# ViliamVadocz/takzero

Measured on NVIDIA B200. Metric: self-play MCTS simulations/sec, 6x6 Tak, higher is better.
Workload: dtype f16

## Files before the change

### takzero_b200/csrc/conv_tcgen05.cuh

```cuda
#pragma once
#include <cuda_bf16.h>
#include <cuda_fp16.h>
#include <stdint.h>
#include <stdio.h>

#include "encode.cuh"

namespace conv {

constexpr int TILE_M = 128;
constexpr int HALO = 8;
constexpr int A_ROWS = TILE_M + 2 * HALO;
constexpr int A_KC_BYTES = A_ROWS * 16;
constexpr int A_STAGE_BYTES = 8 * A_KC_BYTES;
#ifndef TZ_A_STAGES
#define TZ_A_STAGES 4
#endif
#ifndef TZ_B_STAGES
#define TZ_B_STAGES 8
#endif
constexpr int A_STAGES = TZ_A_STAGES;
constexpr int B_KC_BYTES = 128 * 16;
constexpr int B_STAGE_BYTES = 8 * B_KC_BYTES;
constexpr int B_STAGES = TZ_B_STAGES;
constexpr int N_OUT = 256;
constexpr int THREADS = 256;
constexpr int W_EPI0 = 0, W_APROD = 4, W_BPROD = 5, W_MMA = 6, W_ALLOC = 7;
constexpr int MASK_BYTES = 37 * 9 * 16;
constexpr int GATHER_BYTES = 4 * 32 * 32 * 4;
constexpr int SMEM_BYTES =
    A_STAGES * A_STAGE_BYTES + B_STAGES * B_STAGE_BYTES + 4096  + 512  +
    MASK_BYTES + GATHER_BYTES;
static_assert(SMEM_BYTES <= 227 * 1024, "shared memory budget of one CTA");
constexpr int MAX_LAYERS = 48;

struct Layer {
    const __nv_bfloat16* in;
    const TzState* enc_states;
    const __nv_bfloat16* w;
    const float* bias;
    const __nv_bfloat16* residual;
    __nv_bfloat16* out_act;
    const float* head_w;
    float* head_out;
    float* g_out;
    const uint16_t* g_actions;
    const uint32_t* g_ranges;
    const uint16_t* g_perm;
    int g_stride;
    int cin;
    int relu;
    int out_is_residual;
};

struct Params {
    Layer layers[MAX_LAYERS];
    const __nv_bfloat16* dead_after[MAX_LAYERS];
    int n_layers;
    long long rows_set;
    long long set_stride;
    int chunk_min_tiles;
    const int* count_ptr;
    int count_max;
    int n;
    int guard;
    const uint4* masks;
    int f16;
    unsigned* progress;
    unsigned* chunk_done;
    unsigned* status;
    int debug_drop_progress;
    int allow_local;
    int pack;
};

struct Item {
    int chunk, layer, pt;
    int tiles;
    int rows;
};
struct Schedule {
    int chunk_rows;
    int chunk_tiles;
    int rows_used;
    int n_layers;
    int items;
    __host__ __device__ __forceinline__ void init(int count, int nn, int chunk_min_tiles, int layers) {
        rows_used = count * nn;
        const int c1 = count > 0 ? count : 1;
        const int all_tiles = (rows_used + 2 * TILE_M - 1) / (2 * TILE_M);
        const int n_chunks = all_tiles >= 2 * chunk_min_tiles ? all_tiles / chunk_min_tiles : 1;
        const int cp = (c1 + n_chunks - 1) / n_chunks;
        chunk_rows = cp * nn;
        chunk_tiles = (chunk_rows + 2 * TILE_M - 1) / (2 * TILE_M);
        n_layers = layers;
        const int full = rows_used / chunk_rows, rest = rows_used - full * chunk_rows;
        items = (full * chunk_tiles + (rest + 2 * TILE_M - 1) / (2 * TILE_M)) * layers;
// ... 20 lines not shown
    return t;
}
#define CHAIN(cond, layer, kind, k)                                        \
    do {                                                                   \
        if (cond) g_chain[((layer) - 10) * 32 + (kind) * 4 + (k)] = gtime(); \
    } while (0)
#else
#define CHAIN(cond, layer, kind, k)
#endif

#ifdef TZ_DEBUG_TIMING
#define TWAIT(acc, stmt)                 \
    do {                                 \
        const long long t0_ = clock64(); \
        stmt;                            \
        acc += clock64() - t0_;          \
    } while (0)
#else
#define TWAIT(acc, stmt) stmt
#endif

__device__ __forceinline__ uint32_t smem_u32(const void* p) { return (uint32_t)__cvta_generic_to_shared(p); }

__device__ __forceinline__ bool row_position(int pack, int nn, int count, unsigned row, int* q, int* sq) {
    if (pack == 0) {
        *q = (int)(row / (unsigned)nn);
        *sq = (int)(row - (unsigned)*q * (unsigned)nn);
        return true;
    }
    const unsigned tile = row / (unsigned)TILE_M, w = row - tile * (unsigned)TILE_M, b = w / (unsigned)nn;
    *q = (int)(tile * (unsigned)pack + b);
    *sq = (int)(w - b * (unsigned)nn);
    return (int)b < pack && *q < count;
}

__device__ __forceinline__ void mbar_init(uint32_t bar, uint32_t count) {
    asm volatile("mbarrier.init.shared::cta.b64 [%0], %1;" ::"r"(bar), "r"(count));
}
__device__ __forceinline__ void mbar_wait(uint32_t bar, uint32_t parity) {
    asm volatile(
        "{\n\t"
        ".reg .pred p;\n\t"
        "WAIT_%=:\n\t"
        "mbarrier.try_wait.parity.shared::cta.b64 p, [%0], %1;\n\t"
        "@p bra DONE_%=;\n\t"
        "bra WAIT_%=;\n\t"
        "DONE_%=:\n\t"
        "}\n" ::"r"(bar),
        "r"(parity)
        : "memory");
}
__device__ __forceinline__ void mbar_arrive(uint32_t bar) {
    asm volatile("mbarrier.arrive.shared::cta.b64 _, [%0];" ::"r"(bar) : "memory");
}
__device__ __forceinline__ void mbar_arrive_n(uint32_t bar, uint32_t n) {
    asm volatile("mbarrier.arrive.shared::cta.b64 _, [%0], %1;" ::"r"(bar), "r"(n) : "memory");
// ... 106 lines not shown
    asm volatile(
        "tcgen05.commit.cta_group::2.mbarrier::arrive::one.shared::cluster.multicast::cluster.b64 [%0], %1;" ::"r"(bar),
        "h"((uint16_t)3)
        : "memory");
}
__device__ __forceinline__ void tc_mma_pair(uint32_t tmem_d, uint64_t adesc, uint64_t bdesc, uint32_t idesc, uint32_t acc,
                                            const uint4& m0, const uint4& m1) {
    asm volatile(
        "{\n\t"
        ".reg .pred p;\n\t"
        "setp.ne.b32 p, %4, 0;\n\t"
        "tcgen05.mma.cta_group::2.kind::f16 [%0], %1, %2, %3, {%5, %6, %7, %8, %9, %10, %11, %12}, p;\n\t"
        "}\n" ::"r"(tmem_d),
        "l"(adesc), "l"(bdesc), "r"(idesc), "r"(acc), "r"(m0.x), "r"(m0.y), "r"(m0.z), "r"(m0.w), "r"(m1.x), "r"(m1.y),
        "r"(m1.z), "r"(m1.w)
        : "memory");
}


__global__ void __cluster_dims__(2, 1, 1) __launch_bounds__(THREADS, 1) k_conv3x3_pair(const __grid_constant__ Params p) {
    extern __shared__ __align__(128) uint8_t smem[];
    const int warp = threadIdx.x >> 5, lane = threadIdx.x & 31;
    const uint32_t rank = cluster_rank();
    uint8_t* a_smem = smem;
    uint8_t* b_smem = smem + A_STAGES * A_STAGE_BYTES;
    float* s_bias = reinterpret_cast<float*>(b_smem + B_STAGES * B_STAGE_BYTES);
    uint64_t* bars = reinterpret_cast<uint64_t*>(reinterpret_cast<uint8_t*>(s_bias) + 4096);
    const uint32_t bar0 = smem_u32(bars);
    const uint32_t a_full = bar0, a_land = a_full + 8 * A_STAGES, a_empty = a_land + 8 * A_STAGES;
    const uint32_t b_full = a_empty + 8 * A_STAGES, b_land = b_full + 8 * B_STAGES;
    const uint32_t b_empty = b_land + 8 * B_STAGES;
    const uint32_t t_full = b_empty + 8 * B_STAGES, t_empty = t_full + 16;
    uint32_t* tmem_slot = reinterpret_cast<uint32_t*>(bars + 3 * A_STAGES + 3 * B_STAGES + 4);
    uint4* s_masks = reinterpret_cast<uint4*>(reinterpret_cast<uint8_t*>(bars) + 512);
    float* s_gather = reinterpret_cast<float*>(reinterpret_cast<uint8_t*>(s_masks) + MASK_BYTES);

    const int count = p.count_ptr ? *p.count_ptr : p.count_max;
    const int nn = p.n * p.n;
    const int period = p.pack ? TILE_M : nn;
    Schedule sched;
    sched.init(p.pack ? (count + p.pack - 1) / p.pack : count, period, p.chunk_min_tiles, p.n_layers);
    const int items = sched.items;
    const int pair = blockIdx.x >> 1, npairs = gridDim.x >> 1;
    const bool fine = sched.chunk_tiles < 2 * npairs;
    const bool local = p.allow_local && p.n_layers > 1 && (TILE_M % period) == 0 && sched.chunk_tiles <= npairs &&
                       items == sched.chunk_tiles * p.n_layers;
    const int item0 = local ? (pair < sched.chunk_tiles ? pair : items) : pair;
    const int istep = local ? sched.chunk_tiles : npairs;
    const uint32_t a_arrivals = local ? 4u : 1u;

    if (threadIdx.x == 0) {
        for (int i = 0; i < A_STAGES; i++) {
            mbar_init(a_full + 8 * i, 2 * a_arrivals);
            mbar_init(a_land + 8 * i, 1);
            mbar_init(a_empty + 8 * i, 1);
        }
        for (int i = 0; i < B_STAGES; i++) {
            mbar_init(b_full + 8 * i, 2);
            mbar_init(b_land + 8 * i, 1);
            mbar_init(b_empty + 8 * i, 1);
        }
        for (int i = 0; i < 2; i++) {
            mbar_init(t_full + 8 * i, 1);
            mbar_init(t_empty + 8 * i, 8);
        }
        asm volatile("fence.mbarrier_init.release.cluster;" ::: "memory");
    }
    if (warp == W_ALLOC) {
        asm volatile("tcgen05.alloc.cta_group::2.sync.aligned.shared::cta.b32 [%0], %1;" ::"r"(smem_u32(tmem_slot)),
                     "r"(512)
                     : "memory");
        asm volatile("tcgen05.relinquish_alloc_permit.cta_group::2.sync.aligned;" ::: "memory");
    }
    for (int i = threadIdx.x; i < (nn + 1) * 9; i += THREADS) s_masks[i] = p.masks[i];
    tc_fence_before();
    __syncthreads();
    cluster_sync_all();
    tc_fence_after();
    const uint32_t tmem_base = *tmem_slot;
    const uint32_t a_sig = rank == 0 ? a_full : a_land, b_sig = rank == 0 ? b_full : b_land;

    if (warp == W_APROD) {
        int stage = 0, phase = 0;
        for (int item = item0; item < items; item += istep) {
            const Item it = sched.at(item);
            const int layer = it.layer, pt = it.pt;
            const Layer& L = p.layers[layer];
            const int t = pt * 2 + (int)rank;
            if (L.enc_states != nullptr) {
                if (lane == 0) {
                    if (it.chunk >= 2 && p.n_layers > 1)
                        wait_counter(p.chunk_done + it.chunk - 2, 8u * (unsigned)sched.chunk_tiles, p.status);
                    mbar_wait(a_empty + 8 * stage, phase ^ 1);
                }
                __syncwarp();
#ifdef TZ_DEBUG_TIMING
                const long long enc_t0 = clock64();
#endif
                uint8_t* dst = a_smem + stage * A_STAGE_BYTES;
                const int first = t * TILE_M - HALO;
                constexpr int RPL = (A_ROWS + 31) / 32;
                uint64_t stack[RPL];
                uint4 tail[RPL];
                uint32_t hts[RPL];
#pragma unroll
                for (int k = 0; k < RPL; k++) {
                    const int r = lane + 32 * k;
                    const int rel = first + r;
                    hts[k] = 0xffffffffu;
                    stack[k] = 0;
                    tail[k] = make_uint4(0u, 0u, 0u, 0u);
                    if (r < A_ROWS && rel >= 0 && rel < it.rows) {
                        const unsigned grow = (unsigned)(it.chunk * sched.chunk_rows + rel);
                        int q, sq;
                        if (row_position(p.pack, nn, count, grow, &q, &sq)) {
                            const uint8_t* st = reinterpret_cast<const uint8_t*>(L.enc_states + q);
                            stack[k] = *reinterpret_cast<const uint64_t*>(st + 8 * sq);
                            hts[k] = (uint32_t)st[288 + sq] | ((uint32_t)st[324 + sq] << 8) | ((uint32_t)st[360] << 16);
                            tail[k] = *reinterpret_cast<const uint4*>(st + 368);
                        }
                    }
                }
#pragma unroll
                for (int k = 0; k < RPL; k++) {
                    const int r = lane + 32 * k;
                    if (r >= A_ROWS) continue;
                    uint8_t* row = dst + r * 16;
                    if (hts[k] != 0xffffffffu) {
                        const uint64_t ones = enc::square_indicator_bits(stack[k], (int)(hts[k] & 0xff), (int)((hts[k] >> 8) & 0xff),
                                                                         (int)((hts[k] >> 16) & 0xff), p.n);
                        enc::encode_square16_smem(row, A_KC_BYTES, ones, tail[k].y, tail[k].z, tail[k].w, p.n, p.f16);
                    } else {
#pragma unroll
                        for (int kc = 0; kc < 8; kc++) *reinterpret_cast<uint4*>(row + kc * A_KC_BYTES) = make_uint4(0u, 0u, 0u, 0u);
                    }
                }
                asm volatile("fence.proxy.async.shared::cta;" ::: "memory");
                __syncwarp();
                if (lane == 0) {
                    if (rank == 0) mbar_arrive_n(a_sig + 8 * stage, a_arrivals);
                    else mbar_arrive(a_sig + 8 * stage);
                }
#ifdef TZ_DEBUG_TIMING
                if (pair == 0 && rank == 0 && lane == 0 && item < 2 * npairs) printf("encode of one tile: %lld cycles\n", clock64() - enc_t0);
#endif
                if (++stage == A_STAGES) {
                    stage = 0;
                    phase ^= 1;
                }
                continue;
            }
            const int kblocks = L.cin >> 6;
            if (local) continue;
            if (lane == 0) {
                const unsigned need = 8u * (unsigned)layer;
                const unsigned* prog = p.progress + ((size_t)it.chunk * sched.chunk_tiles) * 4;
                const int lo = pt - 1 + (int)rank;
                const __nv_bfloat16* in_base = L.in + (size_t)(it.chunk & 1) * p.set_stride;
                const uint8_t* src_tile =
                    reinterpret_cast<const uint8_t*>(in_base) + (size_t)(p.guard + t * TILE_M - HALO) * 16;
                int st = stage, ph = phase;
                for (int kb = 0; kb < kblocks; kb++) {
                    if (layer > 0 && (fine || kb == 0)) {
                        const int blk = fine ? kb : 3;
                        for (int q = lo; q <= lo + 1; q++)
                            if (q >= 0 && q < it.tiles) wait_counter(prog + q * 4 + blk, need, p.status);
                        fence_proxy_async();
                        CHAIN(pair == 10 && rank == 0 && (layer == 10 || layer == 11), layer, 0, kb);
                    }
                    mbar_wait(a_empty + 8 * st, ph ^ 1);
                    mbar_arrive_expect_tx(a_sig + 8 * st, A_STAGE_BYTES);
                    const uint32_t dst = smem_u32(a_smem + st * A_STAGE_BYTES);
#pragma unroll
                    for (int kc = 0; kc < 8; kc++)
                        bulk_g2s(dst + kc * A_KC_BYTES, src_tile + (size_t)(kb * 8 + kc) * (size_t)p.rows_set * 16,
                                 A_KC_BYTES, a_sig + 8 * st);
                    if (++st == A_STAGES) {
                        st = 0;
                        ph ^= 1;
                    }
                }
            }
            for (int kb = 0; kb < kblocks; kb++)
                if (++stage == A_STAGES) {
                    stage = 0;
                    phase ^= 1;
                }
        }
    } else if (warp == W_BPROD) {
        if (lane == 0) {
            int stage = 0, phase = 0;
            for (int item = item0; item < items; item += istep) {
                const Layer& L = p.layers[sched.at(item).layer];
                const uint8_t* src = reinterpret_cast<const uint8_t*>(L.w) + (size_t)rank * B_STAGE_BYTES;
                const int blocks = (L.cin >> 6) * 9;
                for (int blk = 0; blk < blocks; blk++) {
                    mbar_wait(b_empty + 8 * stage, phase ^ 1);
                    mbar_arrive_expect_tx(b_sig + 8 * stage, B_STAGE_BYTES);
                    bulk_g2s(smem_u32(b_smem + stage * B_STAGE_BYTES), src + (size_t)blk * 2 * B_STAGE_BYTES,
                             B_STAGE_BYTES, b_sig + 8 * stage);
                    if (++stage == B_STAGES) {
                        stage = 0;
                        phase ^= 1;
                    }
                }
            }
        }
    } else if (warp == W_ALLOC) {
        if (rank != 0 && lane == 0) {
            int stage = 0, phase = 0;
            const uint32_t b_full_leader = map_to_rank(b_full, 0);
            for (int item = item0; item < items; item += istep) {
                const int blocks = (p.layers[sched.at(item).layer].cin >> 6) * 9;
                for (int blk = 0; blk < blocks; blk++) {
                    mbar_wait(b_land + 8 * stage, phase);
                    mbar_arrive_cluster(b_full_leader + 8 * stage);
                    if (++stage == B_STAGES) {
                        stage = 0;
                        phase ^= 1;
                    }
                }
            }
        }
    } else if (warp == W_MMA) {
        if (rank != 0) {
            if (lane == 0) {
                int stage = 0, phase = 0;
                const uint32_t a_full_leader = map_to_rank(a_full, 0);
                for (int item = item0; item < items; item += istep) {
                    const Layer& RL = p.layers[sched.at(item).layer];
                    if (local && RL.enc_states == nullptr) break;
                    const int kblocks = RL.cin >> 6;
                    for (int kb = 0; kb < kblocks; kb++) {
                        mbar_wait(a_land + 8 * stage, phase);
                        mbar_arrive_cluster_n(a_full_leader + 8 * stage, a_arrivals);
                        if (++stage == A_STAGES) {
                            stage = 0;
                            phase ^= 1;
                        }
                    }
                }
            }
        } else {
            const uint32_t fmt = p.f16 ? 0u : 1u;
            const uint32_t idesc = (1u << 4) | (fmt << 7) | (fmt << 10) | ((uint32_t)(N_OUT >> 3) << 17) |
                                   ((uint32_t)((2 * TILE_M) >> 4) << 24);
            int a_stage = 0, a_phase = 0, b_stage = 0, b_phase = 0, it = 0;
#ifdef TZ_DEBUG_TIMING
            long long w_t = 0, w_a = 0, w_b = 0, w_a0 = 0;
            const long long mma_start = clock64();
            long long gt_start;
            asm volatile("mov.u64 %0, %%globaltimer;" : "=l"(gt_start));
#endif
            for (int item = item0; item < items; item += istep, it++) {
                const Item wi = sched.at(item);
                const int pt = wi.pt;
                const int kblocks = p.layers[wi.layer].cin >> 6;
                const int acc = it & 1;
                TWAIT(w_t, mbar_wait(t_empty + 8 * acc, ((it >> 1) & 1) ^ 1));
                tc_fence_after();
                const uint32_t tmem_d = tmem_base + acc * N_OUT;
                const uint4* masks0 = s_masks + (p.pack ? (size_t)nn : (size_t)(pt * 2) * TILE_M % nn) * 9;
                const uint4* masks1 = s_masks + (p.pack ? (size_t)nn : (size_t)(pt * 2 + 1) * TILE_M % nn) * 9;
                for (int kb = 0; kb < kblocks; kb++) {
#ifdef TZ_DEBUG_TIMING
                    if (p.layers[wi.layer].enc_states != nullptr)
                        TWAIT(w_a0, mbar_wait(a_full + 8 * a_stage, a_phase));
                    else
#endif
                        TWAIT(w_a, mbar_wait(a_full + 8 * a_stage, a_phase));
                    const uint32_t a_base = smem_u32(a_smem + a_stage * A_STAGE_BYTES);
                    for (int ti = 0; ti < 9; ti++) {
                        const int tap = ti == 0 ? 4 : (ti <= 4 ? ti - 1 : ti);
                        TWAIT(w_b, mbar_wait(b_full + 8 * b_stage, b_phase));
                        tc_fence_after();
                        CHAIN(pair == 10 && lane == 0 && ti == 0 && (wi.layer == 10 || wi.layer == 11), wi.layer, 1, kb);
                        const int off = (tap / 3 - 1) * p.n + (tap % 3 - 1);
                        const uint4 m0 = masks0[tap], m1 = masks1[tap];
                        const uint32_t a_tap = a_base + (HALO + off) * 16;
                        const uint32_t b_base = smem_u32(b_smem + b_stage * B_STAGE_BYTES);
                        if (elect_one()) {
#pragma unroll
                            for (int ks = 0; ks < 4; ks++) {
                                const uint64_t adesc = make_desc(a_tap + ks * 2 * A_KC_BYTES, A_KC_BYTES);
                                const uint64_t bdesc = make_desc(b_base + ks * 2 * B_KC_BYTES, B_KC_BYTES);
                                tc_mma_pair(tmem_d, adesc, bdesc, idesc, (kb | ti | ks) != 0, m0, m1);
                            }
                            tc_commit_pair(b_empty + 8 * b_stage);
                            if (ti == 8) tc_commit_pair(a_empty + 8 * a_stage);
                            if (ti == 8 && kb == kblocks - 1) tc_commit_pair(t_full + 8 * acc);
                            CHAIN(pair == 10 && ti == 8 && kb == kblocks - 1 && (wi.layer == 10 || wi.layer == 11), wi.layer, 3, 1);
                        }
                        __syncwarp();
                        if (++b_stage == B_STAGES) {
                            b_stage = 0;
                            b_phase ^= 1;
                        }
                    }
                    if (++a_stage == A_STAGES) {
                        a_stage = 0;
                        a_phase ^= 1;
                    }
                }
            }
#ifdef TZ_DEBUG_TIMING
            if ((pair == 0 || pair == 40) && lane == 0)
            {
                long long gt_end;
                asm volatile("mov.u64 %0, %%globaltimer;" : "=l"(gt_end));
                printf("pair %d mma: tiles %d total %lld wait_tmem %lld wait_a %lld (encoded tiles %lld) wait_b %lld ns %lld\n",
                       pair, it, clock64() - mma_start, w_t, w_a, w_a0, w_b, gt_end - gt_start);
            }
#endif
        }
    } else if (warp >= W_EPI0 && warp < W_EPI0 + 4) {
        const int wq = warp & 3;
        const uint32_t t_empty_leader = map_to_rank(t_empty, 0);
        const size_t plane = (size_t)p.rows_set * 8;
        float* bias_w = s_bias + wq * N_OUT;
        const uint32_t a_full_leader = map_to_rank(a_full, 0);
        int it = 0, bias_layer = -1, a_consumed = 0;
        for (int item = item0; item < items; item += istep, it++) {
            const Item wi = sched.at(item);
            const int layer = wi.layer, pt = wi.pt;
            const Layer& L = p.layers[layer];
            if (layer != bias_layer) {
                __syncwarp();
#pragma unroll
                for (int j = 0; j < N_OUT / 32; j++) bias_w[lane + 32 * j] = __ldg(L.bias + lane + 32 * j);
                __syncwarp();
                bias_layer = layer;
            }
            const size_t set_off = (size_t)(wi.chunk & 1) * p.set_stride;
            const __nv_bfloat16* residual = L.residual ? L.residual + set_off : nullptr;
            a_consumed += L.cin >> 6;
            const int a_next = a_consumed % A_STAGES;
            const bool to_smem = local && L.out_act != nullptr && layer + 1 < p.n_layers;
            __nv_bfloat16* out_act = L.out_act && (!local || L.out_is_residual) ? L.out_act + set_off : nullptr;
            const float* head_w = L.head_w;
            const int relu = L.relu;
            const int acc = it & 1;
            const int t = pt * 2 + (int)rank;
            const int rel = t * TILE_M + wq * 32 + lane;
            const size_t grow = (size_t)(p.guard + rel) * 8;
            const size_t grel = (size_t)wi.chunk * sched.chunk_rows + (size_t)rel;
            int q_row = 0, sq_row = 0;
            const bool valid = rel < wi.rows && row_position(p.pack, nn, count, (unsigned)grel, &q_row, &sq_row);
            float head_v = 0.0f, head_u = 0.0f;
            float* g_row = nullptr;
            const uint16_t* g_act = nullptr;
            const uint16_t* g_perm = nullptr;
            int g_first = 0, g_count = 0;
            uint32_t g_ch0 = 0, g_ch1 = 0, g_valid = 0, g_blocks = 0;
            int g_q = 0;
            if (L.g_out != nullptr && valid) {
                const int q = q_row, sq = sq_row;
                g_q = q;
                const uint32_t range = L.g_ranges[(size_t)q * 36 + sq];
                g_first = (int)(range & 0xffffu);
                g_count = (int)(range >> 16);
                g_row = L.g_out + (size_t)q * L.g_stride;
                g_act = L.g_actions + (size_t)q * L.g_stride;
                g_perm = L.g_perm ? L.g_perm + (size_t)q * L.g_stride : nullptr;
                for (int m = 0; m < g_count; m++) {
                    const int i = g_perm ? (int)g_perm[g_first + m] : g_first + m;
                    const int ch = enc::move_channel(p.n, g_act[i]);
                    if (ch < 0 || ch >= N_OUT) continue;
                    g_blocks |= 1u << (ch >> 5);
                    if (m < 4) g_ch0 |= (uint32_t)ch << (8 * m);
                    else if (m < 8) g_ch1 |= (uint32_t)ch << (8 * (m - 4));
                    if (m < 8) g_valid |= 1u << m;
                }
            }
            float* stg = s_gather + (wq * 32 + lane) * 32;
            mbar_wait(t_full + 8 * acc, (it >> 1) & 1);
            tc_fence_after();
#ifndef TZ_NO_DISCARD
            if (p.dead_after[layer] != nullptr && !local && p.n_layers > 1) {
                const uint8_t* base = reinterpret_cast<const uint8_t*>(p.dead_after[layer] + set_off) +
                                      (size_t)(p.guard + t * TILE_M + HALO) * 16;
                for (int i = wq * 32 + lane; i < 14 * 32; i += 128) {
                    const int plane_i = i / 14, line_i = i - plane_i * 14;
                    if (t * TILE_M + HALO + 8 * line_i < wi.rows)
                        discard_l2_line(base + (size_t)plane_i * (size_t)p.rows_set * 16 + (size_t)line_i * 128);
                }
            }
#endif
            CHAIN(pair == 10 && rank == 0 && wq == 0 && lane == 0 && (layer == 10 || layer == 11), layer, 3, 0);
            unsigned* prog_tile = p.progress + ((size_t)wi.chunk * sched.chunk_tiles + pt) * 4;
            if (residual != nullptr && layer >= 2 && !local) (void)ld_acquire_gpu(prog_tile + 3);
            const uint32_t taddr = tmem_base + ((uint32_t)(wq * 32) << 16) + acc * N_OUT;
            uint4 rnext[4];
            if (residual && valid) {
#pragma unroll
                for (int j = 0; j < 4; j++) rnext[j] = *reinterpret_cast<const uint4*>(residual + (size_t)j * plane + grow);
            }
#pragma unroll 1
            for (int c0 = 0; c0 < N_OUT; c0 += 32) {
                uint32_t v[32];
                tmem_ld32(taddr + c0, v);
                uint4 rcur[4];
// ... 142 lines not shown
```

### takzero_b200/csrc/nn.cu

```cuda
#include <math.h>
#include <stdio.h>
#include <stdlib.h>
#include <string.h>

#include <string>
#include <type_traits>
#include <vector>

#include "comm.cuh"
#include "conv_tcgen05.cuh"
#include "encode.cuh"
#include "nn.cuh"
#include "planes.cuh"
#include "rnd.cuh"
#include "rules.cuh"

#define WPB TZ_WARPS_PER_BLOCK
#define FILTERS 256
#define CIN_PAD 64
#define SET_HEADER_BYTES 256
#define SET_MAGIC 0x53575a54u

struct SetLayout {
    int layers = 0;
// ... 344 lines not shown
    std::string name;
    const float* data;
    std::vector<long long> shape;
    size_t numel() const {
        size_t k = 1;
        for (long long s : shape) k *= (size_t)s;
        return k;
    }
};

static const HostTensor* find(const std::vector<HostTensor>& ts, const std::string& name) {
    for (const HostTensor& t : ts)
        if (t.name == name) return &t;
    return nullptr;
}

struct ChunkBounds {
    int chunks, chunk_tiles;
};
static ChunkBounds chunk_bounds(int count_max, int nn, int chunk_min_tiles) {
    const int all_tiles = (int)(((long long)count_max * nn + 2 * conv::TILE_M - 1) / (2 * conv::TILE_M));
    ChunkBounds b;
    b.chunks = all_tiles >= 2LL * chunk_min_tiles ? all_tiles / chunk_min_tiles : 1;
    b.chunk_tiles = b.chunks > 1 ? 2 * chunk_min_tiles + 2 : (all_tiles > 0 ? all_tiles : 1);
    return b;
}

static thread_local char g_nn_err[256] = "";
const char* nn_last_error() { return g_nn_err; }
#define NN_FAIL(code, ...)                              \
    do {                                                \
        snprintf(g_nn_err, sizeof(g_nn_err), __VA_ARGS__); \
        return code;                                    \
    } while (0)

static size_t align_up(size_t x, size_t a) { return (x + a - 1) / a * a; }

static void make_layouts(int n, int blocks, SetLayout* lay, RawLayout* raw) {
    const int cin0 = 2 * (2 * n + 3 + 2) + 2, cout_p = 3 + 4 * ((1 << n) - 2);
    lay->layers = 2 * blocks + 2;
    size_t off = SET_HEADER_BYTES, roff = 0;
    for (int l = 0; l < lay->layers; l++) {
        const bool first = l == 0, last = l == lay->layers - 1;
        lay->cin_pad[l] = first ? CIN_PAD : FILTERS;
        lay->w[l] = off;
        off += (size_t)(lay->cin_pad[l] / 64) * 9 * 16384 * 2;
        lay->b[l] = off;
// ... 67 lines not shown
    h->nn = s;
    s->n = n;
    s->blocks = blocks;
    s->in_channels = 2 * (2 * n + 3 + 2) + 2;
    s->out_channels = 3 + 4 * ((1 << n) - 2);
    s->max_positions = h->d.Q;
    make_layouts(n, blocks, &s->lay, &s->raw);
    cudaDeviceGetAttribute(&s->sm_count, cudaDevAttrMultiProcessorCount, h->device);
    auto dalloc = [&](void** p, size_t bytes) -> bool {
        if (cudaMalloc(p, bytes) != cudaSuccess) return false;
        s->allocs.push_back(*p);
        return cudaMemset(*p, 0, bytes) == cudaSuccess;
    };
    {
        s->fused = want_fused;
        const int tiles = h->dbg_chunk_tiles >= 0 ? h->dbg_chunk_tiles : 150;
        s->cfg_chunk_tiles = h->dbg_chunk_tiles;
        const size_t used = (size_t)s->max_positions * nn;
        const int all_tiles = (int)((used + 2 * conv::TILE_M - 1) / (2 * conv::TILE_M));
        s->chunk_min_tiles = (!s->fused || tiles <= 0 || all_tiles < 2 * tiles) ? (1 << 28) : tiles;
        const ChunkBounds cb = chunk_bounds(s->max_positions, nn, s->chunk_min_tiles);
        s->chunk_tiles = cb.chunk_tiles;
        s->max_chunks = cb.chunks;
        s->rows_set = conv::HALO + (size_t)s->chunk_tiles * (2 * conv::TILE_M) + 2 * conv::HALO;
        s->pack = 0;
        if (s->fused && h->dbg_chunk_tiles < 0 && conv::TILE_M % nn != 0) {
            const int per_tile = conv::TILE_M / nn;
            const int tiles = (s->max_positions + per_tile - 1) / per_tile;
            if (tiles <= 2 * (s->sm_count / 2)) {
                s->pack = per_tile;
                const size_t rows = conv::HALO + (size_t)((tiles + 1) / 2) * (2 * conv::TILE_M) + 2 * conv::HALO;
                if (rows > s->rows_set) s->rows_set = rows;
            }
        }
    }
    const size_t act_bytes = 2 * s->rows_set * FILTERS * 2;
    if (dalloc((void**)&s->act_x, 2 * act_bytes)) s->act_t = s->act_x + act_bytes / 2;
    if (!s->act_x ||
        !dalloc((void**)&s->head_feat, (size_t)s->max_positions * nn * 2 * sizeof(float)) ||
        !dalloc((void**)&s->perm, (size_t)s->max_positions * h->d.M * sizeof(uint16_t)) ||
        !dalloc((void**)&s->wset[0], s->lay.total) || !dalloc((void**)&s->wset[1], s->lay.total)) {
        nn_free(h);
        NN_FAIL(TZ_ENOMEM, "cudaMalloc of the network buffers failed");
    }
    {
        std::vector<uint32_t> mk((size_t)(nn + 1) * 9 * 4, 0);
        for (int start = 0; start < nn; start++)
            for (int tap = 0; tap < 9; tap++) {
                const int dy = tap / 3 - 1, dx = tap % 3 - 1;
                for (int i = 0; i < conv::TILE_M; i++) {
                    const int sq = (start + i) % nn, y = sq / n, x = sq % n;
                    const bool off = y + dy < 0 || y + dy >= n || x + dx < 0 || x + dx >= n;
                    if (off) mk[((size_t)start * 9 + tap) * 4 + i / 32] |= 1u << (i % 32);
                }
            }
        for (int tap = 0; tap < 9; tap++) {
            const int dy = tap / 3 - 1, dx = tap % 3 - 1;
            for (int i = 0; i < conv::TILE_M; i++) {
                const int sq = i % nn, y = sq / n, x = sq % n;
                const bool off = i / nn >= conv::TILE_M / nn || y + dy < 0 || y + dy >= n || x + dx < 0 || x + dx >= n;
                if (off) mk[((size_t)nn * 9 + tap) * 4 + i / 32] |= 1u << (i % 32);
            }
        }
        if (!dalloc((void**)&s->masks, mk.size() * 4) ||
            cudaMemcpy(s->masks, mk.data(), mk.size() * 4, cudaMemcpyHostToDevice) != cudaSuccess) {
            nn_free(h);
            NN_FAIL(TZ_ENOMEM, "cudaMalloc masks");
        }
    }
    if (cudaFuncSetAttribute(conv::k_conv3x3_pair, cudaFuncAttributeMaxDynamicSharedMemorySize, conv::SMEM_BYTES) !=
        cudaSuccess) {
        nn_free(h);
        NN_FAIL(TZ_ECUDA, "cudaFuncSetAttribute(k_conv3x3_pair, %d B smem) failed", conv::SMEM_BYTES);
    }
    {
        cudaLaunchConfig_t cfg = {};
        cfg.gridDim = dim3(2 * (s->sm_count / 2));
        cfg.blockDim = dim3(conv::THREADS);
        cfg.dynamicSmemBytes = conv::SMEM_BYTES;
        int clusters = 0;
        if (cudaOccupancyMaxActiveClusters(&clusters, conv::k_conv3x3_pair, &cfg) == cudaSuccess && clusters > 0)
            s->max_pairs = clusters < s->sm_count / 2 ? clusters : s->sm_count / 2;
        else
            s->max_pairs = s->sm_count / 2;
        if (s->pack && (s->max_positions + s->pack - 1) / s->pack > 2 * s->max_pairs) s->pack = 0;
        s->progress_len = (size_t)s->max_chunks * s->chunk_tiles * 4 + s->max_chunks + 16 + (s->pack ? 4 * (size_t)s->max_pairs : 0);
// ... 267 lines not shown
struct Boundary {
    const TzState* states;
    const uint16_t* actions;
    const uint32_t* ranges;
    const uint16_t* perm;
    float* logits;
};

static conv::Layer conv_layer(const NnState* s, int set, int l, const __nv_bfloat16* in, const __nv_bfloat16* residual,
                              __nv_bfloat16* out_act, int relu) {
    conv::Layer L;
    memset(&L, 0, sizeof(L));
    L.in = in;
    L.w = reinterpret_cast<const __nv_bfloat16*>(s->wset[set] + s->lay.w[l]);
    L.bias = reinterpret_cast<const float*>(s->wset[set] + s->lay.b[l]);
    L.residual = residual;
    L.out_act = out_act;
    L.cin = s->lay.cin_pad[l];
    L.relu = relu;
    return L;
}

static cudaError_t launch_layers(tz_handle* h, conv::Params& p, int set, const int* count_ptr, int count_max, size_t rows_set,
                                 int chunk_min_tiles, int pack = 0) {
    const NnState* s = h->nn;
    p.pack = pack;
    const int nn = pack ? conv::TILE_M : s->n * s->n;
    const int units_max = pack ? (count_max + pack - 1) / pack : count_max;
    p.rows_set = (long long)rows_set;
    p.set_stride = (long long)rows_set * FILTERS;
    p.chunk_min_tiles = chunk_min_tiles;
    p.count_ptr = count_ptr;
    p.count_max = count_max;
    p.n = s->n;
    p.guard = conv::HALO;
    p.masks = s->masks;
    p.f16 = s->set_f16[set];
    const int all_tiles = (units_max * nn + 2 * conv::TILE_M - 1) / (2 * conv::TILE_M);
    const ChunkBounds cb = chunk_bounds(units_max, nn, chunk_min_tiles);
    const int chunks = cb.chunks, chunk_tiles = cb.chunk_tiles;
    const size_t counters = (size_t)chunks * chunk_tiles * 4 + chunks;
    p.progress = s->progress;
    p.chunk_done = s->progress + (size_t)chunks * chunk_tiles * 4;
    p.status = h->d.status;
    p.debug_drop_progress = h->dbg_drop_progress;
    const long long items = (long long)all_tiles * p.n_layers;
    const int pairs = items < s->max_pairs ? (items > 0 ? (int)items : 1) : s->max_pairs;
    cudaLaunchConfig_t cfg = {};
    cfg.gridDim = dim3(2 * pairs);
    cfg.blockDim = dim3(conv::THREADS);
    cfg.dynamicSmemBytes = conv::SMEM_BYTES;
// ... 28 lines not shown
    all.back().head_out = s->head_feat;
    all.push_back(conv_layer(s, set, 1 + 2 * s->blocks, s->act_x, nullptr, nullptr, 0));
    all.back().g_out = io.logits;
    all.back().g_actions = io.actions;
    all.back().g_ranges = io.ranges;
    all.back().g_perm = io.perm;
    all.back().g_stride = h->d.M;
    if (upto >= 0 && (size_t)upto < all.size()) all.resize((size_t)upto);
    int launches = 0;
    for (size_t first = 0; first < all.size();) {
        const size_t chunk = s->fused ? all.size() - first : 1;
        conv::Params p;
        for (size_t i = 0; i < chunk; i++) {
            p.layers[i] = all[first + i];
            p.dead_after[i] = nullptr;
        }
        if (chunk == all.size() && upto < 0) {
            for (size_t i = 2; i + 1 < chunk; i += 2) p.dead_after[i] = s->act_t;
            p.dead_after[chunk - 1] = s->act_x;
        }
        p.n_layers = (int)chunk;
        p.allow_local = upto < 0;
        const int pack = p.allow_local && chunk == all.size() ? s->pack : 0;
        if (launch_layers(h, p, set, count_ptr, count_max, s->rows_set, s->chunk_min_tiles, pack) != cudaSuccess) return -1;
        first += chunk;
        launches++;
    }
    return launches;
}

static void launch_novelty(tz_handle* h, const TzState* states, const int* count_ptr, int count_max) {
    NnState* s = h->nn;
    const TzDev& d = h->d;
    const int wblocks = (count_max + WPB - 1) / WPB;
    if (!s->simhash_set) return;
    if (s->novelty == 2)
        k_lcghash<<<wblocks, 32 * WPB, 0, h->stream>>>(states, count_ptr, count_max, d.n, d.half_komi, s->lcghash_init,
                                                       s->simhash_idx);
    else
        k_simhash<<<wblocks, 32 * WPB, 0, h->stream>>>(states, count_ptr, count_max, d.n, d.half_komi, s->simhash_matrix,
                                                       s->simhash_idx);
    h->launches += 1;
}

int nn_forward_queue(tz_handle* h) {
    NnState* s = h->nn;
    if (!s || s->active < 0) return TZ_ENOWEIGHTS;
// ... 240 lines not shown
```

Measured before the change: 1.071 million.

## Add board-row layout for fused conv that skips off-board taps

Adds a 'board' mode to the tcgen05 conv kernel for board sizes that do not divide the tile. Positions are grouped so that each tile covers whole board rows, and the A operand is loaded as three row-shifted regions instead of one haloed strip. For tiles on the top or bottom board row, the weight loads and MMAs of the off-board taps are skipped, which removes wasted tensor-core work and weight traffic. In exchange it uses fewer A/B pipeline stages, adds extra x-masks, disables activation discard in board mode, and adds more per-item index arithmetic. It only activates when pack is 0.

```diff
diff --git a/takzero_b200/csrc/conv_tcgen05.cuh b/takzero_b200/csrc/conv_tcgen05.cuh
--- a/takzero_b200/csrc/conv_tcgen05.cuh
+++ b/takzero_b200/csrc/conv_tcgen05.cuh
@@ -23,14 +23,22 @@
 constexpr int B_KC_BYTES = 128 * 16;
 constexpr int B_STAGE_BYTES = 8 * B_KC_BYTES;
 constexpr int B_STAGES = TZ_B_STAGES;
+constexpr int BR_ROWS = TILE_M + 2;
+constexpr int BR_KC_BYTES = BR_ROWS * 16;
+constexpr int BR_REGION_BYTES = 8 * BR_KC_BYTES;
+constexpr int BR_STAGE_BYTES = 3 * BR_REGION_BYTES;
+constexpr int BR_A_STAGES = 2, BR_B_STAGES = 6;
 constexpr int N_OUT = 256;
 constexpr int THREADS = 256;
 constexpr int W_EPI0 = 0, W_APROD = 4, W_BPROD = 5, W_MMA = 6, W_ALLOC = 7;
-constexpr int MASK_BYTES = 37 * 9 * 16;
+constexpr int MASK_BYTES = (37 + 6) * 9 * 16;
 constexpr int GATHER_BYTES = 4 * 32 * 32 * 4;
+constexpr int AB_BYTES_DENSE = A_STAGES * A_STAGE_BYTES + B_STAGES * B_STAGE_BYTES;
+constexpr int AB_BYTES_BOARD = BR_A_STAGES * BR_STAGE_BYTES + BR_B_STAGES * B_STAGE_BYTES;
+constexpr int AB_BYTES = AB_BYTES_DENSE > AB_BYTES_BOARD ? AB_BYTES_DENSE : AB_BYTES_BOARD;
+static_assert(BR_A_STAGES <= A_STAGES && BR_B_STAGES <= B_STAGES, "barriers are allocated for the dense stage counts");
 constexpr int SMEM_BYTES =
-    A_STAGES * A_STAGE_BYTES + B_STAGES * B_STAGE_BYTES + 4096  + 512  +
-    MASK_BYTES + GATHER_BYTES;
+    AB_BYTES + 4096  + 512  + MASK_BYTES + GATHER_BYTES;
 static_assert(SMEM_BYTES <= 227 * 1024, "shared memory budget of one CTA");
 constexpr int MAX_LAYERS = 48;
 
@@ -72,7 +80,18 @@
     int debug_drop_progress;
     int allow_local;
     int pack;
+    int board;
 };
+
+__host__ __device__ __forceinline__ int board_unit(int n) {
+    int g = 256;
+    for (int a = n; a != 0;) {
+        const int r = g % a;
+        g = a;
+        a = r;
+    }
+    return 256 / g;
+}
 
 struct Item {
     int chunk, layer, pt;
@@ -139,7 +158,17 @@
 
 __device__ __forceinline__ uint32_t smem_u32(const void* p) { return (uint32_t)__cvta_generic_to_shared(p); }
 
-__device__ __forceinline__ bool row_position(int pack, int nn, int count, unsigned row, int* q, int* sq) {
+__device__ __forceinline__ bool row_position(int pack, int board, int n, int count, const Schedule& s, const Item& it,
+                                             int rel, int* q, int* sq) {
+    const int nn = n * n;
+    if (board) {
+        const int per_row = it.rows / n;
+        const int y = rel / per_row, w = rel - y * per_row, pi = w / n;
+        *q = it.chunk * (s.chunk_rows / nn) + pi;
+        *sq = y * n + (w - pi * n);
+        return *q < count;
+    }
+    const unsigned row = (unsigned)(it.chunk * s.chunk_rows + rel);
     if (pack == 0) {
         *q = (int)(row / (unsigned)nn);
         *sq = (int)(row - (unsigned)*q * (unsigned)nn);
@@ -149,6 +178,11 @@
     *q = (int)(tile * (unsigned)pack + b);
     *sq = (int)(w - b * (unsigned)nn);
     return (int)b < pack && *q < count;
+}
+
+__device__ __forceinline__ int board_y(const Item& it, int n) { return it.pt / (it.tiles / n); }
+__device__ __forceinline__ bool tap_off_board(int board, int y, int n, int tap) {
+    return board && ((y == 0 && tap < 3) || (y == n - 1 && tap >= 6));
 }
 
 __device__ __forceinline__ void mbar_init(uint32_t bar, uint32_t count) {
@@ -301,9 +335,11 @@
     extern __shared__ __align__(128) uint8_t smem[];
     const int warp = threadIdx.x >> 5, lane = threadIdx.x & 31;
     const uint32_t rank = cluster_rank();
+    const int board = p.pack == 0 && p.board;
+    const int a_stages = board ? BR_A_STAGES : A_STAGES, b_stages = board ? BR_B_STAGES : B_STAGES;
     uint8_t* a_smem = smem;
-    uint8_t* b_smem = smem + A_STAGES * A_STAGE_BYTES;
-    float* s_bias = reinterpret_cast<float*>(b_smem + B_STAGES * B_STAGE_BYTES);
+    uint8_t* b_smem = smem + (board ? BR_A_STAGES * BR_STAGE_BYTES : A_STAGES * A_STAGE_BYTES);
+    float* s_bias = reinterpret_cast<float*>(smem + AB_BYTES);
     uint64_t* bars = reinterpret_cast<uint64_t*>(reinterpret_cast<uint8_t*>(s_bias) + 4096);
     const uint32_t bar0 = smem_u32(bars);
     const uint32_t a_full = bar0, a_land = a_full + 8 * A_STAGES, a_empty = a_land + 8 * A_STAGES;
@@ -316,9 +352,10 @@
 
     const int count = p.count_ptr ? *p.count_ptr : p.count_max;
     const int nn = p.n * p.n;
-    const int period = p.pack ? TILE_M : nn;
+    const int unit = board ? board_unit(p.n) : 1;
+    const int period = p.pack ? TILE_M : unit * nn;
     Schedule sched;
-    sched.init(p.pack ? (count + p.pack - 1) / p.pack : count, period, p.chunk_min_tiles, p.n_layers);
+    sched.init(p.pack ? (count + p.pack - 1) / p.pack : (count + unit - 1) / unit, period, p.chunk_min_tiles, p.n_layers);
     const int items = sched.items;
     const int pair = blockIdx.x >> 1, npairs = gridDim.x >> 1;
     const bool fine = sched.chunk_tiles < 2 * npairs;
@@ -351,7 +388,7 @@
                      : "memory");
         asm volatile("tcgen05.relinquish_alloc_permit.cta_group::2.sync.aligned;" ::: "memory");
     }
-    for (int i = threadIdx.x; i < (nn + 1) * 9; i += THREADS) s_masks[i] = p.masks[i];
+    for (int i = threadIdx.x; i < (nn + 1 + p.n) * 9; i += THREADS) s_masks[i] = p.masks[i];
     tc_fence_before();
     __syncthreads();
     cluster_sync_all();
@@ -366,6 +403,12 @@
             const int layer = it.layer, pt = it.pt;
             const Layer& L = p.layers[layer];
             const int t = pt * 2 + (int)rank;
+            const int per_row = board ? it.rows / p.n : 0;
+            const int y = board ? board_y(it, p.n) : 0;
+            const int g_lo = board && y > 0 ? 0 : 1, g_hi = board && y < p.n - 1 ? 2 : 1;
+            const int reg_rows = board ? BR_ROWS : A_ROWS, kc_bytes = board ? BR_KC_BYTES : A_KC_BYTES;
+            const int stage_bytes = board ? BR_STAGE_BYTES : A_STAGE_BYTES;
+            const uint32_t tx_bytes = board ? (uint32_t)(g_hi - g_lo + 1) * BR_REGION_BYTES : A_STAGE_BYTES;
             if (L.enc_states != nullptr) {
                 if (lane == 0) {
                     if (it.chunk >= 2 && p.n_layers > 1)
@@ -376,42 +419,44 @@
 #ifdef TZ_DEBUG_TIMING
                 const long long enc_t0 = clock64();
 #endif
-                uint8_t* dst = a_smem + stage * A_STAGE_BYTES;
-                const int first = t * TILE_M - HALO;
-                constexpr int RPL = (A_ROWS + 31) / 32;
-                uint64_t stack[RPL];
-                uint4 tail[RPL];
-                uint32_t hts[RPL];
-#pragma unroll
-                for (int k = 0; k < RPL; k++) {
-                    const int r = lane + 32 * k;
-                    const int rel = first + r;
-                    hts[k] = 0xffffffffu;
-                    stack[k] = 0;
-                    tail[k] = make_uint4(0u, 0u, 0u, 0u);
-                    if (r < A_ROWS && rel >= 0 && rel < it.rows) {
-                        const unsigned grow = (unsigned)(it.chunk * sched.chunk_rows + rel);
-                        int q, sq;
-                        if (row_position(p.pack, nn, count, grow, &q, &sq)) {
-                            const uint8_t* st = reinterpret_cast<const uint8_t*>(L.enc_states + q);
-                            stack[k] = *reinterpret_cast<const uint64_t*>(st + 8 * sq);
-                            hts[k] = (uint32_t)st[288 + sq] | ((uint32_t)st[324 + sq] << 8) | ((uint32_t)st[360] << 16);
-                            tail[k] = *reinterpret_cast<const uint4*>(st + 368);
+#pragma unroll 1
+                for (int g = g_lo; g <= g_hi; g++) {
+                    uint8_t* dst = a_smem + stage * stage_bytes + (board ? g * BR_REGION_BYTES : 0);
+                    const int first = board ? t * TILE_M - 1 + (g - 1) * per_row : t * TILE_M - HALO;
+                    constexpr int RPL = (A_ROWS + 31) / 32;
+                    uint64_t stack[RPL];
+                    uint4 tail[RPL];
+                    uint32_t hts[RPL];
+#pragma unroll
+                    for (int k = 0; k < RPL; k++) {
+                        const int r = lane + 32 * k;
+                        const int rel = first + r;
+                        hts[k] = 0xffffffffu;
+                        stack[k] = 0;
+                        tail[k] = make_uint4(0u, 0u, 0u, 0u);
+                        if (r < reg_rows && rel >= 0 && rel < it.rows) {
+                            int q, sq;
+                            if (row_position(p.pack, board, p.n, count, sched, it, rel, &q, &sq)) {
+                                const uint8_t* st = reinterpret_cast<const uint8_t*>(L.enc_states + q);
+                                stack[k] = *reinterpret_cast<const uint64_t*>(st + 8 * sq);
+                                hts[k] = (uint32_t)st[288 + sq] | ((uint32_t)st[324 + sq] << 8) | ((uint32_t)st[360] << 16);
+                                tail[k] = *reinterpret_cast<const uint4*>(st + 368);
+                            }
                         }
                     }
-                }
-#pragma unroll
-                for (int k = 0; k < RPL; k++) {
-                    const int r = lane + 32 * k;
-                    if (r >= A_ROWS) continue;
-                    uint8_t* row = dst + r * 16;
-                    if (hts[k] != 0xffffffffu) {
-                        const uint64_t ones = enc::square_indicator_bits(stack[k], (int)(hts[k] & 0xff), (int)((hts[k] >> 8) & 0xff),
-                                                                         (int)((hts[k] >> 16) & 0xff), p.n);
-                        enc::encode_square16_smem(row, A_KC_BYTES, ones, tail[k].y, tail[k].z, tail[k].w, p.n, p.f16);
-                    } else {
-#pragma unroll
-                        for (int kc = 0; kc < 8; kc++) *reinterpret_cast<uint4*>(row + kc * A_KC_BYTES) = make_uint4(0u, 0u, 0u, 0u);
+#pragma unroll
+                    for (int k = 0; k < RPL; k++) {
+                        const int r = lane + 32 * k;
+                        if (r >= reg_rows) continue;
+                        uint8_t* row = dst + r * 16;
+                        if (hts[k] != 0xffffffffu) {
+                            const uint64_t ones = enc::square_indicator_bits(stack[k], (int)(hts[k] & 0xff), (int)((hts[k] >> 8) & 0xff),
+                                                                             (int)((hts[k] >> 16) & 0xff), p.n);
+                            enc::encode_square16_smem(row, kc_bytes, ones, tail[k].y, tail[k].z, tail[k].w, p.n, p.f16);
+                        } else {
+#pragma unroll
+                            for (int kc = 0; kc < 8; kc++) *reinterpret_cast<uint4*>(row + kc * kc_bytes) = make_uint4(0u, 0u, 0u, 0u);
+                        }
                     }
                 }
                 asm volatile("fence.proxy.async.shared::cta;" ::: "memory");
@@ -423,7 +468,7 @@
 #ifdef TZ_DEBUG_TIMING
                 if (pair == 0 && rank == 0 && lane == 0 && item < 2 * npairs) printf("encode of one tile: %lld cycles\n", clock64() - enc_t0);
 #endif
-                if (++stage == A_STAGES) {
+                if (++stage == a_stages) {
                     stage = 0;
                     phase ^= 1;
                 }
@@ -435,33 +480,37 @@
                 const unsigned need = 8u * (unsigned)layer;
                 const unsigned* prog = p.progress + ((size_t)it.chunk * sched.chunk_tiles) * 4;
                 const int lo = pt - 1 + (int)rank;
+                const int tiles_row = board ? it.tiles / p.n : 0;
                 const __nv_bfloat16* in_base = L.in + (size_t)(it.chunk & 1) * p.set_stride;
-                const uint8_t* src_tile =
-                    reinterpret_cast<const uint8_t*>(in_base) + (size_t)(p.guard + t * TILE_M - HALO) * 16;
                 int st = stage, ph = phase;
                 for (int kb = 0; kb < kblocks; kb++) {
                     if (layer > 0 && (fine || kb == 0)) {
                         const int blk = fine ? kb : 3;
-                        for (int q = lo; q <= lo + 1; q++)
-                            if (q >= 0 && q < it.tiles) wait_counter(prog + q * 4 + blk, need, p.status);
+                        for (int g = g_lo; g <= g_hi; g++)
+                            for (int q = lo + (g - 1) * tiles_row; q <= lo + 1 + (g - 1) * tiles_row; q++)
+                                if (q >= 0 && q < it.tiles) wait_counter(prog + q * 4 + blk, need, p.status);
                         fence_proxy_async();
                         CHAIN(pair == 10 && rank == 0 && (layer == 10 || layer == 11), layer, 0, kb);
                     }
                     mbar_wait(a_empty + 8 * st, ph ^ 1);
-                    mbar_arrive_expect_tx(a_sig + 8 * st, A_STAGE_BYTES);
-                    const uint32_t dst = smem_u32(a_smem + st * A_STAGE_BYTES);
-#pragma unroll
-                    for (int kc = 0; kc < 8; kc++)
-                        bulk_g2s(dst + kc * A_KC_BYTES, src_tile + (size_t)(kb * 8 + kc) * (size_t)p.rows_set * 16,
-                                 A_KC_BYTES, a_sig + 8 * st);
-                    if (++st == A_STAGES) {
+                    mbar_arrive_expect_tx(a_sig + 8 * st, tx_bytes);
+                    for (int g = g_lo; g <= g_hi; g++) {
+                        const uint32_t dst = smem_u32(a_smem + st * stage_bytes + (board ? g * BR_REGION_BYTES : 0));
+                        const int first = board ? t * TILE_M - 1 + (g - 1) * per_row : t * TILE_M - HALO;
+                        const uint8_t* src = reinterpret_cast<const uint8_t*>(in_base) + (size_t)(p.guard + first) * 16;
+#pragma unroll
+                        for (int kc = 0; kc < 8; kc++)
+                            bulk_g2s(dst + kc * kc_bytes, src + (size_t)(kb * 8 + kc) * (size_t)p.rows_set * 16, kc_bytes,
+                                     a_sig + 8 * st);
+                    }
+                    if (++st == a_stages) {
                         st = 0;
                         ph ^= 1;
                     }
                 }
             }
             for (int kb = 0; kb < kblocks; kb++)
-                if (++stage == A_STAGES) {
+                if (++stage == a_stages) {
                     stage = 0;
                     phase ^= 1;
                 }
@@ -470,15 +519,19 @@
         if (lane == 0) {
             int stage = 0, phase = 0;
             for (int item = item0; item < items; item += istep) {
-                const Layer& L = p.layers[sched.at(item).layer];
+                const Item it = sched.at(item);
+                const Layer& L = p.layers[it.layer];
+                const int y = board ? board_y(it, p.n) : 0;
                 const uint8_t* src = reinterpret_cast<const uint8_t*>(L.w) + (size_t)rank * B_STAGE_BYTES;
                 const int blocks = (L.cin >> 6) * 9;
                 for (int blk = 0; blk < blocks; blk++) {
+                    const int ti = blk % 9;
+                    if (tap_off_board(board, y, p.n, ti == 0 ? 4 : (ti <= 4 ? ti - 1 : ti))) continue;
                     mbar_wait(b_empty + 8 * stage, phase ^ 1);
                     mbar_arrive_expect_tx(b_sig + 8 * stage, B_STAGE_BYTES);
                     bulk_g2s(smem_u32(b_smem + stage * B_STAGE_BYTES), src + (size_t)blk * 2 * B_STAGE_BYTES,
                              B_STAGE_BYTES, b_sig + 8 * stage);
-                    if (++stage == B_STAGES) {
+                    if (++stage == b_stages) {
                         stage = 0;
                         phase ^= 1;
                     }
@@ -490,11 +543,15 @@
             int stage = 0, phase = 0;
             const uint32_t b_full_leader = map_to_rank(b_full, 0);
             for (int item = item0; item < items; item += istep) {
-                const int blocks = (p.layers[sched.at(item).layer].cin >> 6) * 9;
+                const Item it = sched.at(item);
+                const int y = board ? board_y(it, p.n) : 0;
+                const int blocks = (p.layers[it.layer].cin >> 6) * 9;
                 for (int blk = 0; blk < blocks; blk++) {
+                    const int ti = blk % 9;
+                    if (tap_off_board(board, y, p.n, ti == 0 ? 4 : (ti <= 4 ? ti - 1 : ti))) continue;
                     mbar_wait(b_land + 8 * stage, phase);
                     mbar_arrive_cluster(b_full_leader + 8 * stage);
-                    if (++stage == B_STAGES) {
+                    if (++stage == b_stages) {
                         stage = 0;
                         phase ^= 1;
                     }
@@ -513,7 +570,7 @@
                     for (int kb = 0; kb < kblocks; kb++) {
                         mbar_wait(a_land + 8 * stage, phase);
                         mbar_arrive_cluster_n(a_full_leader + 8 * stage, a_arrivals);
-                        if (++stage == A_STAGES) {
+                        if (++stage == a_stages) {
                             stage = 0;
                             phase ^= 1;
                         }
@@ -539,8 +596,15 @@
                 TWAIT(w_t, mbar_wait(t_empty + 8 * acc, ((it >> 1) & 1) ^ 1));
                 tc_fence_after();
                 const uint32_t tmem_d = tmem_base + acc * N_OUT;
-                const uint4* masks0 = s_masks + (p.pack ? (size_t)nn : (size_t)(pt * 2) * TILE_M % nn) * 9;
-                const uint4* masks1 = s_masks + (p.pack ? (size_t)nn : (size_t)(pt * 2 + 1) * TILE_M % nn) * 9;
+                const int y = board ? board_y(wi, p.n) : 0;
+                const uint4* masks0 = s_masks + (p.pack ? (size_t)nn
+                                                        : board ? (size_t)(nn + 1 + (pt * 2) * TILE_M % p.n)
+                                                                : (size_t)(pt * 2) * TILE_M % nn) * 9;
+                const uint4* masks1 = s_masks + (p.pack ? (size_t)nn
+                                                        : board ? (size_t)(nn + 1 + (pt * 2 + 1) * TILE_M % p.n)
+                                                                : (size_t)(pt * 2 + 1) * TILE_M % nn) * 9;
+                const int ti_last = board && y == p.n - 1 ? 5 : 8;
+                const int kc_bytes = board ? BR_KC_BYTES : A_KC_BYTES;
                 for (int kb = 0; kb < kblocks; kb++) {
 #ifdef TZ_DEBUG_TIMING
                     if (p.layers[wi.layer].enc_states != nullptr)
@@ -548,35 +612,41 @@
                     else
 #endif
                         TWAIT(w_a, mbar_wait(a_full + 8 * a_stage, a_phase));
-                    const uint32_t a_base = smem_u32(a_smem + a_stage * A_STAGE_BYTES);
+                    const uint32_t a_base = smem_u32(a_smem + a_stage * (board ? BR_STAGE_BYTES : A_STAGE_BYTES));
                     for (int ti = 0; ti < 9; ti++) {
                         const int tap = ti == 0 ? 4 : (ti <= 4 ? ti - 1 : ti);
+                        if (tap_off_board(board, y, p.n, tap)) continue;
                         TWAIT(w_b, mbar_wait(b_full + 8 * b_stage, b_phase));
                         tc_fence_after();
                         CHAIN(pair == 10 && lane == 0 && ti == 0 && (wi.layer == 10 || wi.layer == 11), wi.layer, 1, kb);
                         const int off = (tap / 3 - 1) * p.n + (tap % 3 - 1);
+#ifdef TZ_DEBUG_UNMASKED
+                        const uint4 m0 = make_uint4(0u, 0u, 0u, 0u), m1 = m0;
+#else
                         const uint4 m0 = masks0[tap], m1 = masks1[tap];
-                        const uint32_t a_tap = a_base + (HALO + off) * 16;
+#endif
+                        const uint32_t a_tap = board ? a_base + (tap / 3) * BR_REGION_BYTES + (tap % 3) * 16
+                                                     : a_base + (HALO + off) * 16;
                         const uint32_t b_base = smem_u32(b_smem + b_stage * B_STAGE_BYTES);
                         if (elect_one()) {
 #pragma unroll
                             for (int ks = 0; ks < 4; ks++) {
-                                const uint64_t adesc = make_desc(a_tap + ks * 2 * A_KC_BYTES, A_KC_BYTES);
+                                const uint64_t adesc = make_desc(a_tap + ks * 2 * kc_bytes, kc_bytes);
                                 const uint64_t bdesc = make_desc(b_base + ks * 2 * B_KC_BYTES, B_KC_BYTES);
                                 tc_mma_pair(tmem_d, adesc, bdesc, idesc, (kb | ti | ks) != 0, m0, m1);
                             }
                             tc_commit_pair(b_empty + 8 * b_stage);
-                            if (ti == 8) tc_commit_pair(a_empty + 8 * a_stage);
-                            if (ti == 8 && kb == kblocks - 1) tc_commit_pair(t_full + 8 * acc);
+                            if (ti == ti_last) tc_commit_pair(a_empty + 8 * a_stage);
+                            if (ti == ti_last && kb == kblocks - 1) tc_commit_pair(t_full + 8 * acc);
                             CHAIN(pair == 10 && ti == 8 && kb == kblocks - 1 && (wi.layer == 10 || wi.layer == 11), wi.layer, 3, 1);
                         }
                         __syncwarp();
-                        if (++b_stage == B_STAGES) {
+                        if (++b_stage == b_stages) {
                             b_stage = 0;
                             b_phase ^= 1;
                         }
                     }
-                    if (++a_stage == A_STAGES) {
+                    if (++a_stage == a_stages) {
                         a_stage = 0;
                         a_phase ^= 1;
                     }
@@ -622,9 +692,8 @@
             const int t = pt * 2 + (int)rank;
             const int rel = t * TILE_M + wq * 32 + lane;
             const size_t grow = (size_t)(p.guard + rel) * 8;
-            const size_t grel = (size_t)wi.chunk * sched.chunk_rows + (size_t)rel;
             int q_row = 0, sq_row = 0;
-            const bool valid = rel < wi.rows && row_position(p.pack, nn, count, (unsigned)grel, &q_row, &sq_row);
+            const bool valid = rel < wi.rows && row_position(p.pack, board, p.n, count, sched, wi, rel, &q_row, &sq_row);
             float head_v = 0.0f, head_u = 0.0f;
             float* g_row = nullptr;
             const uint16_t* g_act = nullptr;
@@ -655,7 +724,7 @@
             mbar_wait(t_full + 8 * acc, (it >> 1) & 1);
             tc_fence_after();
 #ifndef TZ_NO_DISCARD
-            if (p.dead_after[layer] != nullptr && !local && p.n_layers > 1) {
+            if (p.dead_after[layer] != nullptr && !local && !board && p.n_layers > 1) {
                 const uint8_t* base = reinterpret_cast<const uint8_t*>(p.dead_after[layer] + set_off) +
                                       (size_t)(p.guard + t * TILE_M + HALO) * 16;
                 for (int i = wq * 32 + lane; i < 14 * 32; i += 128) {
diff --git a/takzero_b200/csrc/nn.cu b/takzero_b200/csrc/nn.cu
--- a/takzero_b200/csrc/nn.cu
+++ b/takzero_b200/csrc/nn.cu
@@ -390,7 +390,7 @@
     const int all_tiles = (int)(((long long)count_max * nn + 2 * conv::TILE_M - 1) / (2 * conv::TILE_M));
     ChunkBounds b;
     b.chunks = all_tiles >= 2LL * chunk_min_tiles ? all_tiles / chunk_min_tiles : 1;
-    b.chunk_tiles = b.chunks > 1 ? 2 * chunk_min_tiles + 2 : (all_tiles > 0 ? all_tiles : 1);
+    b.chunk_tiles = b.chunks > 1 ? 2 * chunk_min_tiles + 2 + nn / (2 * conv::TILE_M) : (all_tiles > 0 ? all_tiles : 1);
     return b;
 }
 
@@ -504,6 +504,12 @@
         const ChunkBounds cb = chunk_bounds(s->max_positions, nn, s->chunk_min_tiles);
         s->chunk_tiles = cb.chunk_tiles;
         s->max_chunks = cb.chunks;
+        if (s->fused && conv::TILE_M % nn != 0) {
+            const int unit = conv::board_unit(n);
+            const ChunkBounds bb = chunk_bounds((s->max_positions + unit - 1) / unit, unit * nn, s->chunk_min_tiles);
+            if (bb.chunk_tiles > s->chunk_tiles) s->chunk_tiles = bb.chunk_tiles;
+            if (bb.chunks > s->max_chunks) s->max_chunks = bb.chunks;
+        }
         s->rows_set = conv::HALO + (size_t)s->chunk_tiles * (2 * conv::TILE_M) + 2 * conv::HALO;
         s->pack = 0;
         if (s->fused && h->dbg_chunk_tiles < 0 && conv::TILE_M % nn != 0) {
@@ -526,7 +532,7 @@
         NN_FAIL(TZ_ENOMEM, "cudaMalloc of the network buffers failed");
     }
     {
-        std::vector<uint32_t> mk((size_t)(nn + 1) * 9 * 4, 0);
+        std::vector<uint32_t> mk((size_t)(nn + 1 + n) * 9 * 4, 0);
         for (int start = 0; start < nn; start++)
             for (int tap = 0; tap < 9; tap++) {
                 const int dy = tap / 3 - 1, dx = tap % 3 - 1;
@@ -544,6 +550,14 @@
                 if (off) mk[((size_t)nn * 9 + tap) * 4 + i / 32] |= 1u << (i % 32);
             }
         }
+        for (int x0 = 0; x0 < n; x0++)
+            for (int tap = 0; tap < 9; tap++) {
+                const int dx = tap % 3 - 1;
+                for (int i = 0; i < conv::TILE_M; i++) {
+                    const int x = (x0 + i) % n;
+                    if (x + dx < 0 || x + dx >= n) mk[((size_t)(nn + 1 + x0) * 9 + tap) * 4 + i / 32] |= 1u << (i % 32);
+                }
+            }
         if (!dalloc((void**)&s->masks, mk.size() * 4) ||
             cudaMemcpy(s->masks, mk.data(), mk.size() * 4, cudaMemcpyHostToDevice) != cudaSuccess) {
             nn_free(h);
@@ -857,11 +871,13 @@
 }
 
 static cudaError_t launch_layers(tz_handle* h, conv::Params& p, int set, const int* count_ptr, int count_max, size_t rows_set,
-                                 int chunk_min_tiles, int pack = 0) {
+                                 int chunk_min_tiles, int pack = 0, int board = 0) {
     const NnState* s = h->nn;
     p.pack = pack;
-    const int nn = pack ? conv::TILE_M : s->n * s->n;
-    const int units_max = pack ? (count_max + pack - 1) / pack : count_max;
+    p.board = pack ? 0 : board;
+    const int unit = p.board ? conv::board_unit(s->n) : 1;
+    const int nn = pack ? conv::TILE_M : unit * s->n * s->n;
+    const int units_max = pack ? (count_max + pack - 1) / pack : (count_max + unit - 1) / unit;
     p.rows_set = (long long)rows_set;
     p.set_stride = (long long)rows_set * FILTERS;
     p.chunk_min_tiles = chunk_min_tiles;
@@ -936,7 +952,9 @@
         p.n_layers = (int)chunk;
         p.allow_local = upto < 0;
         const int pack = p.allow_local && chunk == all.size() ? s->pack : 0;
-        if (launch_layers(h, p, set, count_ptr, count_max, s->rows_set, s->chunk_min_tiles, pack) != cudaSuccess) return -1;
+        const int board = p.allow_local && chunk == all.size() && conv::TILE_M % (s->n * s->n) != 0;
+        if (launch_layers(h, p, set, count_ptr, count_max, s->rows_set, s->chunk_min_tiles, pack, board) != cudaSuccess)
+            return -1;
         first += chunk;
         launches++;
     }
```

Result: slower. 985,500, median of 6 (-7.9%).
